# citibeth/spsparse

Hardware: AMD Instinct MI355X
Metric: nnz(C)/s for C=A*A SpGEMM (higher is better)
Workload: dtype f64

## Files before the change

### spsparse_amd/csrc/capi.hip

```cpp
#include "internal.h"

#include <cstdio>
#include <cstdlib>
#include <cstring>
#include <algorithm>
#include <exception>
#include <vector>

using namespace spsamd;

#define API_GUARD(ctx, ...)                                                         \
	if ((ctx)->busy) { (ctx)->last_error = "context busy: a streamed multiply is delivering on it"; return SPSAMD_EINVAL; } \
	try { __VA_ARGS__ }                                                             \
	catch (const spsamd::Error &e) { (ctx)->last_error = e.msg; return e.code; }    \
	catch (const std::bad_alloc &) { (ctx)->last_error = "host allocation failed"; return SPSAMD_ENOMEM; } \
	catch (const std::exception &e) { (ctx)->last_error = e.what(); return SPSAMD_EINVAL; }

extern "C" const char *spsamd_version(void) { return "spsparse_amd 0.2 (gfx950)"; }

extern "C" int spsamd_ctx_create(spsamd_ctx **out, int device, void *hip_stream)
{
	if (!out) return SPSAMD_EINVAL;
	*out = nullptr;
	int ndev = 0;
	if (hipGetDeviceCount(&ndev) != hipSuccess || ndev == 0) { (void)hipGetLastError(); return SPSAMD_ENODEVICE; }
	if (device < 0) { if (hipGetDevice(&device) != hipSuccess) return SPSAMD_ENODEVICE; }
	if (device >= ndev) return SPSAMD_ENODEVICE;
	if (hipSetDevice(device) != hipSuccess) return SPSAMD_ENODEVICE;
	spsamd_ctx *c = new (std::nothrow) spsamd_ctx();
	if (!c) return SPSAMD_ENOMEM;
	c->device = device;
	hipDeviceProp_t prop;
	if (hipGetDeviceProperties(&prop, device) == hipSuccess) c->num_cu = prop.multiProcessorCount;
	if (hip_stream) { c->stream = (hipStream_t)hip_stream; c->own_stream = false; }
	else {
		if (hipStreamCreateWithFlags(&c->stream, hipStreamNonBlocking) != hipSuccess) { delete c; return SPSAMD_EHIP; }
		c->own_stream = true;
	}
	for (auto &e : c->ev) if (hipEventCreate(&e) != hipSuccess) { spsamd_ctx_destroy(c); return SPSAMD_EHIP; }
	for (auto &e : c->ev2) if (hipEventCreate(&e) != hipSuccess) { spsamd_ctx_destroy(c); return SPSAMD_EHIP; }
	if (hipStreamCreateWithFlags(&c->side, hipStreamNonBlocking) != hipSuccess) { spsamd_ctx_destroy(c); return SPSAMD_EHIP; }
	for (auto &e : c->ev_side) if (hipEventCreateWithFlags(&e, hipEventDisableTiming) != hipSuccess) { spsamd_ctx_destroy(c); return SPSAMD_EHIP; }
	if (hipStreamCreateWithFlags(&c->side2, hipStreamNonBlocking) != hipSuccess) { spsamd_ctx_destroy(c); return SPSAMD_EHIP; }
	for (auto &e : c->ev_side2) if (hipEventCreateWithFlags(&e, hipEventDisableTiming) != hipSuccess) { spsamd_ctx_destroy(c); return SPSAMD_EHIP; }
	static const char *const knobs[] = {"window", "cell_cap", "dense_min", "no_tiles", "xcd", "emit_path", "light_path", "no_wmajor", "direct_min", "tiles_v1", "long_cap", "long_dense_min", "index_budget_mb", "trace", "light_two_pass", "spmm_path", "spmm_long_min", "add_path", "masked_path", "sampled_path", "select_path", "extract_path", "reduce_path", "emult_path", "tile_walk", "solve_path", "solve_row", "solve_fuse_rows", "factor_path", "factor_row", "factor_fuse_rows", "factor_serial_work", "factor_lds_row", "color_path", "color_row", "color_fuse_rows", "color_wave_deg"};
	static const char *const envs[] = {"SPSAMD_W", "SPSAMD_CELL_CAP", "SPSAMD_DENSE_MIN", "SPSAMD_NO_TILES", "SPSAMD_XCD", "SPSAMD_EMIT_PATH", "SPSAMD_LIGHT_PATH", "SPSAMD_NO_WMAJOR", "SPSAMD_DIRECT_MIN", "SPSAMD_TILES_V1", "SPSAMD_LONG_CAP", "SPSAMD_LONG_DENSE_MIN", "SPSAMD_INDEX_BUDGET_MB", "SPSAMD_TRACE", "SPSAMD_LIGHT_TWO_PASS", "SPSAMD_SPMM_PATH", "SPSAMD_SPMM_LONG_MIN", "SPSAMD_ADD_PATH", "SPSAMD_MASKED_PATH", "SPSAMD_SAMPLED_PATH", "SPSAMD_SELECT_PATH", "SPSAMD_EXTRACT_PATH", "SPSAMD_REDUCE_PATH", "SPSAMD_EMULT_PATH", "SPSAMD_TILE_WALK", "SPSAMD_SOLVE_PATH", "SPSAMD_SOLVE_ROW", "SPSAMD_SOLVE_FUSE_ROWS", "SPSAMD_FACTOR_PATH", "SPSAMD_FACTOR_ROW", "SPSAMD_FACTOR_FUSE_ROWS", "SPSAMD_FACTOR_SERIAL_WORK", "SPSAMD_FACTOR_LDS_ROW", "SPSAMD_COLOR_PATH", "SPSAMD_COLOR_ROW", "SPSAMD_COLOR_FUSE_ROWS", "SPSAMD_COLOR_WAVE_DEG"};
	static_assert(sizeof knobs / sizeof knobs[0] == sizeof envs / sizeof envs[0], "one environment variable per knob");
	for (size_t k = 0; k < sizeof knobs / sizeof knobs[0]; ++k)
		if (const char *e = getenv(envs[k])) (void)spsamd_ctx_set_tuning(c, knobs[k], atol(e));
#ifdef SPSAMD_ABLATIONS
	if (const char *e = getenv("SPSAMD_DBG")) c->tune.dbg = atoi(e);
#endif
	*out = c;
	return SPSAMD_OK;
}

extern "C" int spsamd_ctx_set_tuning(spsamd_ctx *c, const char *name, long value)
{
	if (!c || !name) return SPSAMD_EINVAL;
	if (c->busy) { c->last_error = "context busy: a streamed multiply is delivering on it"; return SPSAMD_EINVAL; }
	struct { const char *n; int *p; } tab[] = {
		{"window", &c->tune.window}, {"cell_cap", &c->tune.cell_cap}, {"dense_min", &c->tune.dense_min},
		{"no_tiles", &c->tune.no_tiles}, {"xcd", &c->tune.xcd}, {"emit_path", &c->tune.emit_path},
		{"light_path", &c->tune.light_path}, {"no_wmajor", &c->tune.no_wmajor}, {"direct_min", &c->tune.direct_min}, {"tiles_v1", &c->tune.tiles_v1}, {"long_cap", &c->tune.long_cap}, {"long_dense_min", &c->tune.long_dense_min}, {"index_budget_mb", &c->tune.index_budget_mb}, {"trace", &c->tune.trace}, {"light_two_pass", &c->tune.light_two_pass},
		{"spmm_path", &c->tune.spmm_path}, {"spmm_long_min", &c->tune.spmm_long_min}, {"add_path", &c->tune.add_path},
		{"masked_path", &c->tune.masked_path}, {"sampled_path", &c->tune.sampled_path}, {"select_path", &c->tune.select_path},
		{"extract_path", &c->tune.extract_path}, {"reduce_path", &c->tune.reduce_path}, {"emult_path", &c->tune.emult_path},
		{"tile_walk", &c->tune.tile_walk}, {"solve_path", &c->tune.solve_path}, {"solve_row", &c->tune.solve_row},
		{"solve_fuse_rows", &c->tune.solve_fuse_rows}, {"factor_path", &c->tune.factor_path}, {"factor_row", &c->tune.factor_row},
		{"factor_fuse_rows", &c->tune.factor_fuse_rows}, {"factor_serial_work", &c->tune.factor_serial_work},
		{"factor_lds_row", &c->tune.factor_lds_row}, {"color_path", &c->tune.color_path}, {"color_row", &c->tune.color_row},
		{"color_fuse_rows", &c->tune.color_fuse_rows}, {"color_wave_deg", &c->tune.color_wave_deg},
	};
	for (auto &t : tab) if (!std::strcmp(t.n, name)) { *t.p = (int)value; return SPSAMD_OK; }
	c->last_error = std::string("unknown tuning knob: ") + name;
	return SPSAMD_EINVAL;
}

extern "C" void spsamd_ctx_destroy(spsamd_ctx *c)
{
	if (!c) return;
	(void)hipSetDevice(c->device);
	if (c->stream) (void)hipStreamSynchronize(c->stream);
	if (c->side) (void)hipStreamSynchronize(c->side);
	if (c->side2) (void)hipStreamSynchronize(c->side2);
	c->arena.release();
	c->out[0].release(); c->out[1].release();
	c->rowstat_n.release(); c->rowstat_s.release(); c->rowstat_h.release();
	if (c->pinned) (void)hipHostFree(c->pinned);
	if (c->stream_pinned) (void)hipHostFree(c->stream_pinned);
	for (auto &e : c->ev) if (e) (void)hipEventDestroy(e);
	for (auto &e : c->ev2) if (e) (void)hipEventDestroy(e);
	for (auto &e : c->ev_side) if (e) (void)hipEventDestroy(e);
	for (auto &e : c->ev_side2) if (e) (void)hipEventDestroy(e);
	if (c->side) (void)hipStreamDestroy(c->side);
	if (c->side2) (void)hipStreamDestroy(c->side2);
	if (c->own_stream && c->stream) (void)hipStreamDestroy(c->stream);
	delete c;
}

extern "C" const char *spsamd_last_error(const spsamd_ctx *c) { return c ? c->last_error.c_str() : "null context"; }

extern "C" int spsamd_ctx_reserve(spsamd_ctx *c, size_t workspace_bytes, size_t output_tuples)
{
	if (!c) return SPSAMD_EINVAL;
	API_GUARD(c,
		SPS_HIP(hipSetDevice(c->device));
		if (workspace_bytes) c->arena.reserve(workspace_bytes);
		if (output_tuples) {
			OutSet &o = c->out[c->cur_out];
			o.i.ensure(output_tuples * sizeof(int32_t));
			o.j.ensure(output_tuples * sizeof(int32_t));
			o.v.ensure(output_tuples * sizeof(double));
		}
		return SPSAMD_OK;
	)
}

bool spsamd::same_operand(const spsamd_coo *a, const spsamd_coo *b)
{
	return a->idx0 == b->idx0 && a->idx1 == b->idx1 && a->val == b->val && a->nnz == b->nnz &&
		a->shape0 == b->shape0 && a->shape1 == b->shape1 && a->sort0 == b->sort0 && a->mem == b->mem;
}

int spsamd::multiply_body(spsamd_ctx *c, double C,
	const spsamd_vec *scalei, const spsamd_coo *A, char transpose_A,
	const spsamd_vec *scalej, const spsamd_coo *B, char transpose_B,
	const spsamd_vec *scalek, int duplicate_policy, int zero_nan,
	int sink_kind, int sink_flags, spsamd_result *res, const char *what, bool arena_ready, const OperandParts *parts, bool b_rank1)
{
	check_sink_args(duplicate_policy, sink_kind);
	std::memset(res, 0, sizeof(*res));
	const bool permute = (sink_flags & SPSAMD_SINK_PERMUTE) && sink_kind == SPSAMD_SINK_COO;
	const ProductFrame f(A, transpose_A, B, transpose_B, permute);
	const int a0 = f.a0, bk = f.bk, bj = f.bj;
	res->shape0 = f.shape0; res->shape1 = f.shape1;
	f.check_inner(what);
	if (product_is_empty(C, scalei, A, scalej, B, scalek)) return SPSAMD_OK;

	SPS_HIP(hipSetDevice(c->device));
	if (!arena_ready) c->arena.reset();
	hipStream_t st = c->stream;
	SPS_HIP(hipEventRecord(c->ev[EV_BEGIN], st));
	{ const spsamd_coo *ops[2] = {A, B}; pick_output_set(c, ops, 2); }
	MultiplyArgs a;
	a.C = C; a.sink_kind = sink_kind; a.sink_flags = sink_flags;
	if (parts) { a.pa = parts->pa; a.pb = parts->pb; a.b_ready = parts->b_ready; a.static_walk = true; }
	Prepared *hp = nullptr;
	consolidate_operand(c, A, a0, a0, duplicate_policy, zero_nan, &a.A, &hp);
	if (hp) a.pa = hp;
	if (a0 == bk && same_operand(A, B) && (!zero_nan || hp)) { a.B = a.A; if (a.pa) a.pb = a.pa; }
	else { consolidate_operand(c, B, bk, b_rank1 ? bk : bj, duplicate_policy, zero_nan, &a.B, &hp); if (hp) a.pb = hp; }
	if (sink_kind == SPSAMD_SINK_COO) c->own[c->cur_out].sort0 = -1;
	upload_scale(c, scalei, f.nrow, "scalei", &a.si);
	upload_scale(c, scalej, f.inner, "scalej", &a.sj);
// ... 462 lines not shown
```

### spsparse_amd/csrc/internal.h

```cpp
#pragma once

#include <hip/hip_runtime.h>
#include <stdint.h>
#include <stddef.h>
#include <string>
#include <vector>

#include "../../include/spsparse_amd.h"

namespace spsamd {


struct Error {
	int code;
	std::string msg;
};

#define SPS_HIP(call)                                                              \
	do {                                                                           \
		hipError_t e_ = (call);                                                    \
		if (e_ != hipSuccess)                                                      \
			throw ::spsamd::Error{SPSAMD_EHIP, std::string(#call) + ": " + hipGetErrorString(e_)}; \
	} while (0)

#define SPS_LAUNCH_CHECK() SPS_HIP(hipGetLastError())


struct Arena {
	struct Slab { char *p; size_t cap; size_t used; };
	std::vector<Slab> slabs;
	size_t high_water = 0;
	size_t call_used = 0;

	void *alloc(size_t bytes);
	struct Mark { size_t nslabs, used, call_used; };
	Mark mark() const { return Mark{slabs.size(), slabs.empty() ? 0 : slabs.back().used, call_used}; }
	void rewind(const Mark &m);
	void reset();
	void release();
	void reserve(size_t bytes);
	template <class T> T *get(size_t n) { return (T *)alloc(n * sizeof(T)); }
};

struct DevBuf {
	void *p = nullptr;
	size_t cap = 0;
	void ensure(size_t bytes);
	void release();
	bool holds(const void *q) const { return p && q && (const char *)q >= (const char *)p && (const char *)q < (const char *)p + cap; }
};

struct OutSet {
	DevBuf i, j, v;
	bool holds(const void *q) const { return i.holds(q) || j.holds(q) || v.holds(q); }
	void release() { i.release(); j.release(); v.release(); }
};

struct Tuning {
	int window = 0;
	int cell_cap = 0;
	int dense_min = 0;
	int no_tiles = 0;
	int xcd = 2;
	int emit_path = 0;
	int light_path = 0;
	int light_two_pass = 0;
	int no_wmajor = 0;
	int tiles_v1 = 0;
	int long_cap = 0;
	int long_dense_min = 0;
	int direct_min = 0;
	int trace = 0;
	int index_budget_mb = 0;
	int spmm_path = 0;
	int spmm_long_min = 0;
	int add_path = 0;
	int masked_path = 0;
	int sampled_path = 0;
	int select_path = 0;
	int extract_path = 0;
	int reduce_path = 0;
	int tile_walk = 0;
	int emult_path = 0;
	int solve_path = 0;
	int solve_row = 0;
	int solve_fuse_rows = 0;
	int factor_path = 0;
	int factor_row = 0;
	int factor_fuse_rows = 0;
	int factor_serial_work = 0;
	int factor_lds_row = 0;
	int color_path = 0;
	int color_row = 0;
	int color_fuse_rows = 0;
	int color_wave_deg = 0;
#ifdef SPSAMD_ABLATIONS
	int dbg = 0;
#endif
};
}

struct spsamd_ctx {
	int device = 0;
	spsamd::Tuning tune;
	hipStream_t stream = nullptr;
	bool own_stream = false;
	spsamd::Arena arena;
	spsamd::OutSet out[2];
	int cur_out = 0;
	struct OwnResult { const int32_t *d0 = nullptr, *d1 = nullptr; const double *v = nullptr; uint64_t nnz = 0, shape0 = 0, shape1 = 0; int sort0 = -1; } own[2];
	spsamd::DevBuf rowstat_n, rowstat_s, rowstat_h;
	void *pinned = nullptr;
	size_t pinned_cap = 0;
	std::string last_error;
	hipEvent_t ev[10] = {};
	hipEvent_t ev2[3] = {};
	hipStream_t side = nullptr;
	hipEvent_t ev_side[2] = {};
	hipStream_t side2 = nullptr;
	hipEvent_t ev_side2[2] = {};
	bool wm_pending = false, sort_pending = false;
	void join_side(bool wm, bool sort);
	int num_cu = 256;
	void *host_staging(size_t bytes);
	bool busy = false;
	void *stream_pinned = nullptr;
	size_t stream_pinned_cap = 0;
};

namespace spsamd {

struct SideScope {
	SideScope(spsamd_ctx *c, int which, bool record_fork);
	~SideScope();
	SideScope(const SideScope &) = delete;
	SideScope &operator=(const SideScope &) = delete;
private:
	spsamd_ctx *c;
	hipStream_t main, side;
	hipEvent_t join;
};

enum Ev {
	EV_NONE = -1,
	EV_BEGIN = 0,
	EV_CONSOLIDATED = 1,
	EV_SYMBOLIC = 2,
	EV_N0 = 3,
	EV_N1 = 4,
	EV_N2 = 5,
	EV_N3 = 6,
	EV_END = 7,
	EV_N4 = 8,
// ... 328 lines not shown
```

### spsparse_amd/csrc/k_dense.hip

```cpp
#include "spgemm_host.h"
#include "bank_layout.h"

namespace spsamd {


#ifndef DENSE_SCAN_BATCH
#define DENSE_SCAN_BATCH 8
#endif
#ifndef DENSE_SCAN_XCHG
#define DENSE_SCAN_XCHG 1
#endif
template <int W, int NT, int MODE, bool PAT, bool PLAIN>
__global__ __launch_bounds__(NT, 4) void k_dense(const Cell *cells, uint32_t ncell, const uint32_t *xb, RowMeta m,
	const uint32_t *widx, uint64_t kstride, uint64_t wstride, uint32_t narrow, EmitParams ep, SinkParams sk, uint32_t *claim_ctr)
{
	constexpr int NW = NT / 64;
	constexpr int NGRP = W / 64;
	constexpr int GPW = NGRP / NW;
	constexpr uint32_t WSHIFT = W == 8192 ? 13 : 14;
	constexpr int R = DENSE_R;
	constexpr int NWORD = W / 64;
	constexpr int WPL = NWORD / 64;
	constexpr int SB = DENSE_SCAN_BATCH < GPW ? DENSE_SCAN_BATCH : GPW;
	static_assert(GPW % SB == 0, "whole batches");
	static_assert(!PLAIN || (!PAT && MODE != MODE_COUNT), "PLAIN: STORE and DIGEST without EXACT_PATTERN");
	__shared__ double acc[MODE == MODE_COUNT ? 1 : W + 64];
	__shared__ __attribute__((aligned(16))) uint8_t ctouch[MODE == MODE_COUNT ? W : 16];
	__shared__ uint32_t s_cpref[NT + 1];
	__shared__ uint2 s_cse[NT];
	__shared__ double s_caval[NT];
	__shared__ unsigned long long s_bmask[NWORD];
	__shared__ uint32_t s_scrL[2][NW], s_scrN[2][NW];
	__shared__ uint32_t s_wcnt[NW + 1];
	__shared__ PatCell s_pat;
	__shared__ unsigned long long s_u64[2 * NW];
	__shared__ double s_f64[NW];
	__shared__ uint32_t s_claim[4];

	const unsigned tid = threadIdx.x, lane = lane_id();
	const unsigned wv = (unsigned)__builtin_amdgcn_readfirstlane((int)wave_id());
	const double CLEAN = (PAT && MODE != MODE_COUNT) ? -0.0 : 0.0;
	if (MODE == MODE_COUNT) { for (int q = tid; q < W / 16; q += NT) reinterpret_cast<uint4 *>(ctouch)[q] = make_uint4(0, 0, 0, 0); }
	else for (int q = tid; q < W + 64; q += NT) acc[q] = CLEAN;
	for (int q = tid; q < NWORD; q += NT) s_bmask[q] = 0ull;
	const bool plain = PLAIN || (PAT && emit_plain(ep));
	const unsigned long long laneK = (unsigned long long)lane * 0x9E3779B97F4A7C15ull;
	unsigned long long d_cnt = 0, d_hash = 0; double d_sum = 0;
	PatAcc pat; pat_init(pat);
	if (tid == 0) pat_reset(&s_pat);
	uint32_t flip = 0;
	STAMP_BEGIN();

	constexpr uint32_t NONE = 0xFFFFFFFFu;
	const bool claimed = claim_ctr != nullptr && xb != nullptr && !ABL(ep, 16);
	const CellWalk walk = cell_walk(claimed ? nullptr : xb, ncell);
	const uint32_t stride = walk.stride, cend = walk.end;
	const uint32_t clast = ncell ? ncell - 1 : 0;
	uint32_t part = blockIdx.x & 7u, tried = 0;
	auto claim_resolve = [&](uint32_t got) -> uint32_t {
		while (true) {
			if (got < xb[part + 1]) return got;
			if (++tried >= 8u) return NONE;
			part = (part + 1u) & 7u;
			got = atomicAdd(&claim_ctr[part * 32u], 1u);
		}
	};
	uint32_t i0, i1, i2;
	if (claimed) {
		if (tid == 0) {
			for (int q = 0; q < 3; ++q) s_claim[q] = tried >= 8u ? NONE : claim_resolve(atomicAdd(&claim_ctr[part * 32u], 1u));
			s_claim[3] = NONE;
		}
		__syncthreads();
		i0 = s_claim[0]; i1 = s_claim[1]; i2 = NONE;
	} else {
		i0 = walk.first < cend ? walk.first : NONE;
		i1 = i0 != NONE && i0 + stride < cend ? i0 + stride : NONE;
		i2 = i1 != NONE && i1 + stride < cend ? i1 + stride : NONE;
	}
	i0 = (uint32_t)__builtin_amdgcn_readfirstlane((int)i0); i1 = (uint32_t)__builtin_amdgcn_readfirstlane((int)i1); i2 = (uint32_t)__builtin_amdgcn_readfirstlane((int)i2);
	const uint32_t zlane = cell_pend_zero();
	Cell rec1 = cells[min(i0, clast)];
	CellPend pend2 = cell_pend_load(cells, min(i1, clast), zlane);
	uint32_t nlo, nlen; double na;
	auto seg_bounds = [&](int32_t k, uint32_t w, uint32_t &lo, uint32_t &hi) {
		const uint32_t *bw = widx + (uint64_t)(uint32_t)k * kstride + (uint64_t)w * wstride;
		lo = bw[0]; hi = bw[1];
	};
	{
		const uint32_t e = rec1.beg + tid;
		const bool act = i0 != NONE && e < rec1.end;
		const uint32_t ec = e < rec1.end ? e : rec1.beg;
		uint32_t lo, hi;
		seg_bounds(m.acol[ec], rec1.wa, lo, hi);
		na = m.aval[ec];
		nlo = lo; nlen = act ? hi - lo : 0u;
	}
	int32_t nkA; double naA;
	{
		const uint32_t e1 = rec1.beg + NT + tid;
		const uint32_t e1c = e1 < rec1.end ? e1 : rec1.beg;
		nkA = m.acol[e1c]; naA = m.aval[e1c];
	}
	__syncthreads();
	uint32_t iter = 0;
	for (; i0 != NONE; ++iter, i0 = i1, i1 = i2, i2 = (claimed || i2 == NONE || i2 + stride >= cend) ? (claimed ? i2 : NONE) : i2 + stride) {
		const Cell cell = rec1;
		const uint32_t w = cell.wa;
		const uint32_t beg = cell.beg, end = cell.end;
		const int32_t rowid = cell.rowid;
		double a_scale = 1.0;
		if constexpr (!PLAIN) a_scale = row_scale(ep, rowid);
		const uint32_t wbase = w << WSHIFT;
		uint32_t lo = nlo, len = nlen; double a = na;
		rec1 = cell_from_pend(pend2);
		if (!claimed) pend2 = cell_pend_load(cells, min(i2, clast), zlane);
		const uint32_t ne = rec1.beg + tid;
		const bool nact = i1 != NONE && ne < rec1.end;
		const uint32_t nec = ne < rec1.end ? ne : rec1.beg;
		const int32_t nk = m.acol[nec];
		na = m.aval[nec];
		int32_t kA = nkA; double aA = naA;
		{
			const uint32_t e1 = rec1.beg + NT + tid;
			const uint32_t e1c = e1 < rec1.end ? e1 : rec1.beg;
			nkA = m.acol[e1c]; naA = m.aval[e1c];
		}

		STAMP_COUNT(8);
		uint32_t pnseg = 0;
		for (uint32_t chunk = beg; chunk < end; chunk += NT) {
			STAMP_COUNT(9);
			uint32_t lo2, hi2; double a2;
			{
				seg_bounds(kA, w, lo2, hi2);
				a2 = aA;
				if (chunk + NT + tid >= end) hi2 = lo2;
				const uint32_t e2 = chunk + 2 * NT + tid;
				const uint32_t e2c = e2 < end ? e2 : beg;
				kA = m.acol[e2c]; aA = m.aval[e2c];
			}
			const uint32_t items = (len + R - 1) / R;
			const uint32_t inc = wave_inclusive_scan_u32(items);
			const uint64_t nzm = __ballot(len != 0);
			const uint32_t wrank = (uint32_t)__popcll(nzm & lanemask_lt());
			if (lane == 63) s_scrL[flip][wv] = inc;
			if (lane == 0) s_scrN[flip][wv] = (uint32_t)__popcll(nzm);
			STAMP(0);
			lds_barrier();
			STAMP(1);
			if (claimed && chunk == beg) {
				i2 = (uint32_t)__builtin_amdgcn_readfirstlane((int)s_claim[2 + (iter & 1u)]);
				pend2 = cell_pend_load(cells, min(i2, clast), zlane);
			}
			uint32_t baseL = 0, baseN = 0, total = 0, nzc = 0;
#pragma unroll
			for (int q = 0; q < NW; ++q) {
				const uint32_t l = s_scrL[flip][q], n = s_scrN[flip][q];
				if (q < (int)wv) { baseL += l; baseN += n; }
				total += l; nzc += n;
			}
			flip ^= 1u;
			total = (uint32_t)__builtin_amdgcn_readfirstlane((int)total);
			nzc = (uint32_t)__builtin_amdgcn_readfirstlane((int)nzc);
			const uint32_t myfirst = baseL + inc - items;
			if (len) {
				const uint32_t rank = baseN + wrank;
				s_cpref[rank] = myfirst;
				s_cse[rank] = make_uint2(lo, lo + len);
				s_caval[rank] = a;
				if (myfirst < (uint32_t)W) atomicOr(reinterpret_cast<uint32_t *>(s_bmask) + (myfirst >> 5), 1u << (myfirst & 31u));
			}
			if (ABL(ep, 8)) total = 0;
			if (total == 0) { lo = lo2; len = hi2 - lo2; a = a2; continue; }
			if (ep.ordered && MODE != MODE_COUNT) {
				lds_barrier();
				for (uint32_t q = 0; q < nzc; ++q) {
					const uint2 se = s_cse[q];
					const double aq = s_caval[q];
					for (uint32_t t = se.x + tid; t < se.y; t += NT) {
						const BTup bt = m.btup[t];
						const uint32_t slot = dense_phys((uint32_t)bt.col - wbase);
						acc[slot] = acc[slot] + aq * btup_val(bt);
					}
					lds_barrier();
				}
				for (int q = tid; q < NWORD; q += NT) s_bmask[q] = 0ull;
				lo = lo2; len = hi2 - lo2; a = a2;
				continue;
			}
			uint32_t Q0 = 0;
			for (uint32_t pb = 0; pb < total; pb += W) {
				const uint32_t pe = min(total, pb + (uint32_t)W);
				if (pb) {
					lds_barrier();
					for (int q = tid; q < NWORD; q += NT) s_bmask[q] = 0ull;
					lds_barrier();
					if (len && myfirst >= pb && myfirst < pe) atomicOr(&s_bmask[(myfirst - pb) >> 6], 1ull << ((myfirst - pb) & 63u));
				}
				STAMP(2);
				lds_barrier();
				STAMP(3);
				unsigned long long mw[WPL]; uint32_t pre[WPL];
				uint32_t run = Q0;
#pragma unroll
				for (int x = 0; x < WPL; ++x) {
					mw[x] = s_bmask[x * 64 + lane];
					const uint32_t cnt = (uint32_t)__popcll(mw[x]);
					const uint32_t incl = wave_inclusive_scan_u32(cnt);
					pre[x] = run + incl - cnt;
					run += (uint32_t)__builtin_amdgcn_readlane((int)incl, 63);
				}
				const uint32_t nsteps = (pe - pb + NT - 1) / NT;
				auto lookup = [&](uint32_t step, uint32_t &obp, uint32_t &onv, double &oav) {
					const uint32_t b = step * NW + wv;
					const uint32_t t = pb + (b << 6) + lane;
					const bool ok = t < pe;
					uint32_t mlo = 0, mhi = 0, pr = 0;
#pragma unroll
					for (int x = 0; x < WPL; ++x) {
						if ((b >> 6) == (uint32_t)x) {
							mlo = (uint32_t)__builtin_amdgcn_readlane((int)(uint32_t)mw[x], (int)(b & 63u));
							mhi = (uint32_t)__builtin_amdgcn_readlane((int)(uint32_t)(mw[x] >> 32), (int)(b & 63u));
							pr = (uint32_t)__builtin_amdgcn_readlane((int)pre[x], (int)(b & 63u));
						}
					}
					if (ABL(ep, 128)) { obp = (t * R) & 0xFFFFFu; onv = ok ? R : 0u; oav = 1.0; return; }
					const uint32_t s1lo = (mlo >> 1) | (mhi << 31), s1hi = mhi >> 1;
					const uint32_t qs = pr + (mlo & 1u) - 1u;
					uint32_t q = qs + __builtin_amdgcn_mbcnt_hi(s1hi, __builtin_amdgcn_mbcnt_lo(s1lo, 0u));
					q = min(q, nzc - 1u);
					const uint2 se = s_cse[q];
					obp = se.x + (t - s_cpref[q]) * R;
					onv = ok ? min((uint32_t)R, se.y - obp) : 0u;
					oav = s_caval[q];
				};
				const char *bbase = reinterpret_cast<const char *>(m.btup);
				auto fetch = [&](uint32_t bp_) -> BPiece {
					if (ABL(ep, 64)) bp_ &= 0xFFFFu;
					if (narrow) return *reinterpret_cast<const BPiece *>(bbase + (uint32_t)((bp_ << 3) + (bp_ << 2)));
					return *reinterpret_cast<const BPiece *>(bbase + (uint64_t)bp_ * 12u);
				};
				auto accumulate = [&](const BPiece &piece, uint32_t nv_, double av_) {
#pragma unroll
					for (int u = 0; u < R; ++u) {
						const uint32_t col = ABL(ep, 64) ? (piece.w[3 * u] & (W - 1)) : piece.w[3 * u] - wbase;
						const uint32_t slot = (uint32_t)u < nv_ ? (MODE == MODE_COUNT ? col : dense_phys(col)) : (uint32_t)W + lane;
						if (ABL(ep, 32)) { if (piece.w[3 * u + 2] == 0x7FF12345u) acc[MODE == MODE_COUNT ? 0 : slot] = av_; }
						else if (MODE == MODE_COUNT) { if ((uint32_t)u < nv_) ctouch[slot] = (uint8_t)1; }
						else {
							const double pv = av_ * __hiloint2double((int)piece.w[3 * u + 2], (int)piece.w[3 * u + 1]);
							atomicAdd(&acc[slot], pv);
							if (PAT && (uint32_t)u < nv_) pat_note(pat, pv);
						}
					}
				};
				STAMP(4);
#if DENSE_DEPTH == 2
				uint32_t bp0, nv0, bp1 = 0, nv1 = 0; double av0, av1 = 0.0;
				lookup(0, bp0, nv0, av0);
				BPiece p0 = fetch(bp0), p1 = p0;
				if (nsteps > 1) lookup(1, bp1, nv1, av1);
				for (uint32_t step = 0; step < nsteps; ++step) {
					STAMP_COUNT(10);
					if (step + 1 < nsteps) p1 = fetch(bp1);
					uint32_t bp2 = 0, nv2 = 0; double av2 = 0.0;
					if (step + 2 < nsteps) lookup(step + 2, bp2, nv2, av2);
					accumulate(p0, nv0, av0);
					p0 = p1; nv0 = nv1; av0 = av1;
					bp1 = bp2; nv1 = nv2; av1 = av2;
				}
#else
				uint32_t bp, nv; double av;
				lookup(0, bp, nv, av);
				for (uint32_t step = 0; step < nsteps; ++step) {
					STAMP_COUNT(10);
					const BPiece piece = fetch(bp);
					uint32_t nbp = bp, nnv = 0; double nav = 0.0;
					if (step + 1 < nsteps) lookup(step + 1, nbp, nnv, nav);
					accumulate(piece, nv, av);
					bp = nbp; nv = nnv; av = nav;
				}
#endif
				Q0 = run;
				STAMP(5);
			}
			if (PAT) { pat_publish(pat, &s_pat); pnseg += nzc; }
			lds_barrier();
			STAMP(6);
			for (int q = tid; q < NWORD; q += NT) s_bmask[q] = 0ull;
			lo = lo2; len = hi2 - lo2; a = a2;
		}
		{
			uint32_t l2, h2;
			seg_bounds(nk, rec1.wa, l2, h2);
			nlo = l2; nlen = nact ? h2 - l2 : 0u;
		}
		if (ABL(ep, 16)) continue;
		STAMP(0);
		uint32_t claim_pending = NONE;
		if (claimed && tid == 0 && tried < 8u) claim_pending = atomicAdd(&claim_ctr[part * 32u], 1u);
		const double pthr = PAT ? pat_threshold(&s_pat, pnseg) : -1.0;
		const uint32_t pbeg = beg, pend = end;
		double v[MODE == MODE_STORE ? GPW : 1];
		uint64_t nzmask[MODE == MODE_STORE ? GPW : 1];
		uint32_t wcount = 0;
		constexpr unsigned long long MIXK = 0x9E3779B97F4A7C15ull;
		unsigned long long X0 = ((((unsigned long long)(uint32_t)rowid) << 32) | (unsigned long long)(wbase + wv * GPW * 64u)) * MIXK;
		X0 = ((unsigned long long)(uint32_t)__builtin_amdgcn_readfirstlane((int)(uint32_t)(X0 >> 32)) << 32) |
			(unsigned long long)(uint32_t)__builtin_amdgcn_readfirstlane((int)(uint32_t)X0);
		double r_sum = 0;
		unsigned long long r_hash = 0;
		if constexpr (MODE == MODE_COUNT) {
			static_assert(W / 16 == NT, "sixteen flag bytes per thread");
			uint32_t cnt = 0;
			{
				uint4 *cw = reinterpret_cast<uint4 *>(ctouch);
				const uint4 x = cw[tid];
				const uint32_t xs[4] = {x.x, x.y, x.z, x.w};
				if (x.x | x.y | x.z | x.w) {
					cw[tid] = make_uint4(0, 0, 0, 0);
#pragma unroll
					for (int q = 0; q < 4; ++q) {
						if (!ep.sk_pos) cnt += (uint32_t)__popc(xs[q]);
						else {
#pragma unroll
							for (int b = 0; b < 4; ++b)
								if (((xs[q] >> (8 * b)) & 1u) && col_allowed(ep, (int32_t)(wbase + tid * 16u + (uint32_t)(4 * q + b)))) ++cnt;
						}
					}
				}
			}
			wcount = (uint32_t)wave_reduce_sum((unsigned long long)cnt);
		} else {
		auto slot_of = [&](int gi) -> uint32_t {
			const int grp = wv * GPW + gi;
			return grp * 64 + (lane ^ (uint32_t)__builtin_amdgcn_readfirstlane((int)dense_swz((uint32_t)grp)));
		};
		double xs[SB];
#pragma unroll
		for (int gi = 0; gi < GPW; ++gi) {
			if (gi % SB == 0) {
#if DENSE_SCAN_XCHG
				unsigned long long *acc64 = reinterpret_cast<unsigned long long *>(acc);
#pragma unroll
				for (int q = 0; q < SB; ++q) xs[q] = __longlong_as_double((long long)atomicExch(&acc64[slot_of(gi + q)], (unsigned long long)__double_as_longlong(CLEAN)));
#else
#pragma unroll
				for (int q = 0; q < SB; ++q) xs[q] = acc[slot_of(gi + q)];
#pragma unroll
				for (int q = 0; q < SB; ++q) acc[slot_of(gi + q)] = CLEAN;
#endif
				__builtin_amdgcn_sched_barrier(0);
			}
			const int grp = wv * GPW + gi;
			const int32_t col = (int32_t)(wbase + grp * 64 + lane);
			double x = xs[gi % SB];
			if (PAT) {
				const bool touched = __double_as_longlong(x) != (long long)0x8000000000000000ull;
				x = pat_fix_wave(touched && !(fabs(x) > pthr), x, col, m, pbeg, pend);
			}
			const bool ok = emit_test<PLAIN>(plain, ep, a_scale, col, x);
			const uint64_t mk = __ballot(ok);
			wcount += (uint32_t)__popcll(mk);
			if (MODE == MODE_STORE) { v[gi] = x; nzmask[gi] = mk; }
			if (MODE == MODE_DIGEST) {
				unsigned long long h = X0 + laneK;
				h ^= h >> 29;
				r_hash += ok ? h : 0ull;
				if (plain && !PAT) r_sum += x;
				else r_sum += ok ? x : 0.0;
				X0 += 64ull * MIXK;
			}
		}
		}
		if (MODE == MODE_DIGEST) {
			if (lane == 0) d_cnt += wcount;
			d_sum += r_sum;
			d_hash += r_hash;
			if (sk.row_nnz) {
				double rs = wave_reduce_sum(r_sum);
				r_hash = wave_reduce_sum(r_hash);
				if (lane == 0 && wcount) { atomicAdd((unsigned long long *)&sk.row_nnz[rowid], (unsigned long long)wcount); atomicAdd(&sk.row_sum[rowid], rs); atomicAdd(&sk.row_hash[rowid], r_hash); }
			}
		} else {
			if (lane == 0) s_wcnt[wv] = wcount;
			__syncthreads();
			uint32_t wbefore = 0, wtotal = 0;
#pragma unroll
			for (int q = 0; q < NW; ++q) { uint32_t t = s_wcnt[q]; if (q < (int)wv) wbefore += t; wtotal += t; }
			if (MODE == MODE_COUNT) {
				if (tid == 0) sk.segcount[cell.seg] = wtotal;
			} else {
				int64_t o = sk.segoff[cell.seg] + wbefore;
#pragma unroll
				for (int gi = 0; gi < GPW; ++gi) {
					uint64_t mk = nzmask[gi];
					if ((mk >> lane) & 1ull) {
						int64_t oo = o + __popcll(mk & lanemask_lt());
						sk.out_i[oo] = rowid;
						sk.out_j[oo] = (int32_t)(wbase + (wv * GPW + gi) * 64 + lane);
						sk.out_v[oo] = v[gi];
					}
					o += __popcll(mk);
				}
				if (tid == 0) sk.segactual[cell.seg] = wtotal;
			}
			__syncthreads();
		}
		STAMP(7);
		if (PAT) { lds_barrier(); if (tid == 0) pat_reset(&s_pat); }
		if (claimed && tid == 0) s_claim[2 + ((iter + 1u) & 1u)] = tried < 8u ? claim_resolve(claim_pending) : NONE;
	}
	STAMP_FLUSH();
	if (MODE == MODE_DIGEST) digest_flush<NT>(sk.digest, d_cnt, d_hash, d_sum, s_u64, s_f64);
}

__global__ void k_claim_init(const uint32_t *xb, uint32_t *ctr)
{
	if (threadIdx.x < 8) ctr[threadIdx.x * 32u] = xb[threadIdx.x];
}

template <int MODE>
void launch_heavy_dense(spsamd_ctx *c, const Heavy &hv, const RowMeta &m0, const EmitParams &ep, const SinkParams &sk)
{
	if (!hv.ncell[CLS_DENSE]) return;
	uint32_t *claim = nullptr;
	if (c->tune.xcd == 2 && hv.xb[CLS_DENSE]) {
		claim = c->arena.get<uint32_t>(8 * 32);
		k_claim_init<<<dim3(1), dim3(64), 0, c->stream>>>(hv.xb[CLS_DENSE], claim);
		SPS_LAUNCH_CHECK();
	}
	RowMeta m = m0;
	const uint32_t *widx = hv.bwin;
	uint64_t kstride = hv.nwin1, wstride = 1;
	if (hv.wptr) { widx = hv.wptr; kstride = 1; wstride = hv.nrowb; m.btup = hv.btw; }
	const uint32_t narrow = hv.narrow();
	unsigned grid = std::min<unsigned>(hv.ncell[CLS_DENSE], (unsigned)c->num_cu * (hv.W != 8192 ? 1u : (MODE == MODE_COUNT ? 3u : 2u)));
	if (grid >= 64) grid &= ~7u;
	const SinkParams &sks = stamps_sink(c, sk, grid);
	auto go = [&](auto w, auto nt, auto pat, auto pln) {
		k_dense<decltype(w)::value, decltype(nt)::value, MODE, decltype(pat)::value, decltype(pln)::value><<<dim3(grid), dim3(decltype(nt)::value), 0, c->stream>>>(hv.cells[CLS_DENSE], hv.ncell[CLS_DENSE], hv.xb[CLS_DENSE], m, widx, kstride, wstride, narrow, ep, sks, claim);
	};
	auto go_pat = [&](auto w, auto nt) {
		if (ep.pattern) return go(w, nt, std::true_type{}, std::false_type{});
		if constexpr (MODE != MODE_COUNT) { if (emit_plain(ep)) return go(w, nt, std::false_type{}, std::true_type{}); }
		go(w, nt, std::false_type{}, std::false_type{});
	};
	if (hv.W == 8192) go_pat(std::integral_constant<int, 8192>{}, std::integral_constant<int, 512>{});
	else go_pat(std::integral_constant<int, 16384>{}, std::integral_constant<int, 1024>{});
	SPS_LAUNCH_CHECK();
	static const char *const nm[11] = {"pre-B1", "B1wait", "compact", "B2wait", "tables", "steps", "B3wait", "scanout", "cells", "chunks", "steps#"};
	stamps_report(c, sks, grid, "k_dense", nm, 11, 8);
}

template void launch_heavy_dense<MODE_COUNT>(spsamd_ctx *, const Heavy &, const RowMeta &, const EmitParams &, const SinkParams &);
template void launch_heavy_dense<MODE_STORE>(spsamd_ctx *, const Heavy &, const RowMeta &, const EmitParams &, const SinkParams &);
template void launch_heavy_dense<MODE_DIGEST>(spsamd_ctx *, const Heavy &, const RowMeta &, const EmitParams &, const SinkParams &);

}
```

Before: 163.1 billion.

## Batch multiple A-chunks into one dense expansion group with double-buffered bitmask

New measurement: 164.4 billion (median of 6 runs). No clear change (+0.8%).

```diff
diff --git a/spsparse_amd/csrc/capi.hip b/spsparse_amd/csrc/capi.hip
--- a/spsparse_amd/csrc/capi.hip
+++ b/spsparse_amd/csrc/capi.hip
@@ -43,8 +43,8 @@
 	for (auto &e : c->ev_side) if (hipEventCreateWithFlags(&e, hipEventDisableTiming) != hipSuccess) { spsamd_ctx_destroy(c); return SPSAMD_EHIP; }
 	if (hipStreamCreateWithFlags(&c->side2, hipStreamNonBlocking) != hipSuccess) { spsamd_ctx_destroy(c); return SPSAMD_EHIP; }
 	for (auto &e : c->ev_side2) if (hipEventCreateWithFlags(&e, hipEventDisableTiming) != hipSuccess) { spsamd_ctx_destroy(c); return SPSAMD_EHIP; }
-	static const char *const knobs[] = {"window", "cell_cap", "dense_min", "no_tiles", "xcd", "emit_path", "light_path", "no_wmajor", "direct_min", "tiles_v1", "long_cap", "long_dense_min", "index_budget_mb", "trace", "light_two_pass", "spmm_path", "spmm_long_min", "add_path", "masked_path", "sampled_path", "select_path", "extract_path", "reduce_path", "emult_path", "tile_walk", "solve_path", "solve_row", "solve_fuse_rows", "factor_path", "factor_row", "factor_fuse_rows", "factor_serial_work", "factor_lds_row", "color_path", "color_row", "color_fuse_rows", "color_wave_deg"};
-	static const char *const envs[] = {"SPSAMD_W", "SPSAMD_CELL_CAP", "SPSAMD_DENSE_MIN", "SPSAMD_NO_TILES", "SPSAMD_XCD", "SPSAMD_EMIT_PATH", "SPSAMD_LIGHT_PATH", "SPSAMD_NO_WMAJOR", "SPSAMD_DIRECT_MIN", "SPSAMD_TILES_V1", "SPSAMD_LONG_CAP", "SPSAMD_LONG_DENSE_MIN", "SPSAMD_INDEX_BUDGET_MB", "SPSAMD_TRACE", "SPSAMD_LIGHT_TWO_PASS", "SPSAMD_SPMM_PATH", "SPSAMD_SPMM_LONG_MIN", "SPSAMD_ADD_PATH", "SPSAMD_MASKED_PATH", "SPSAMD_SAMPLED_PATH", "SPSAMD_SELECT_PATH", "SPSAMD_EXTRACT_PATH", "SPSAMD_REDUCE_PATH", "SPSAMD_EMULT_PATH", "SPSAMD_TILE_WALK", "SPSAMD_SOLVE_PATH", "SPSAMD_SOLVE_ROW", "SPSAMD_SOLVE_FUSE_ROWS", "SPSAMD_FACTOR_PATH", "SPSAMD_FACTOR_ROW", "SPSAMD_FACTOR_FUSE_ROWS", "SPSAMD_FACTOR_SERIAL_WORK", "SPSAMD_FACTOR_LDS_ROW", "SPSAMD_COLOR_PATH", "SPSAMD_COLOR_ROW", "SPSAMD_COLOR_FUSE_ROWS", "SPSAMD_COLOR_WAVE_DEG"};
+	static const char *const knobs[] = {"window", "cell_cap", "dense_min", "no_tiles", "xcd", "emit_path", "light_path", "no_wmajor", "direct_min", "tiles_v1", "long_cap", "long_dense_min", "index_budget_mb", "trace", "light_two_pass", "spmm_path", "spmm_long_min", "add_path", "masked_path", "sampled_path", "select_path", "extract_path", "reduce_path", "emult_path", "tile_walk", "solve_path", "solve_row", "solve_fuse_rows", "factor_path", "factor_row", "factor_fuse_rows", "factor_serial_work", "factor_lds_row", "color_path", "color_row", "color_fuse_rows", "color_wave_deg", "dense_groups"};
+	static const char *const envs[] = {"SPSAMD_W", "SPSAMD_CELL_CAP", "SPSAMD_DENSE_MIN", "SPSAMD_NO_TILES", "SPSAMD_XCD", "SPSAMD_EMIT_PATH", "SPSAMD_LIGHT_PATH", "SPSAMD_NO_WMAJOR", "SPSAMD_DIRECT_MIN", "SPSAMD_TILES_V1", "SPSAMD_LONG_CAP", "SPSAMD_LONG_DENSE_MIN", "SPSAMD_INDEX_BUDGET_MB", "SPSAMD_TRACE", "SPSAMD_LIGHT_TWO_PASS", "SPSAMD_SPMM_PATH", "SPSAMD_SPMM_LONG_MIN", "SPSAMD_ADD_PATH", "SPSAMD_MASKED_PATH", "SPSAMD_SAMPLED_PATH", "SPSAMD_SELECT_PATH", "SPSAMD_EXTRACT_PATH", "SPSAMD_REDUCE_PATH", "SPSAMD_EMULT_PATH", "SPSAMD_TILE_WALK", "SPSAMD_SOLVE_PATH", "SPSAMD_SOLVE_ROW", "SPSAMD_SOLVE_FUSE_ROWS", "SPSAMD_FACTOR_PATH", "SPSAMD_FACTOR_ROW", "SPSAMD_FACTOR_FUSE_ROWS", "SPSAMD_FACTOR_SERIAL_WORK", "SPSAMD_FACTOR_LDS_ROW", "SPSAMD_COLOR_PATH", "SPSAMD_COLOR_ROW", "SPSAMD_COLOR_FUSE_ROWS", "SPSAMD_COLOR_WAVE_DEG", "SPSAMD_DENSE_GROUPS"};
 	static_assert(sizeof knobs / sizeof knobs[0] == sizeof envs / sizeof envs[0], "one environment variable per knob");
 	for (size_t k = 0; k < sizeof knobs / sizeof knobs[0]; ++k)
 		if (const char *e = getenv(envs[k])) (void)spsamd_ctx_set_tuning(c, knobs[k], atol(e));
@@ -71,6 +71,7 @@
 		{"factor_fuse_rows", &c->tune.factor_fuse_rows}, {"factor_serial_work", &c->tune.factor_serial_work},
 		{"factor_lds_row", &c->tune.factor_lds_row}, {"color_path", &c->tune.color_path}, {"color_row", &c->tune.color_row},
 		{"color_fuse_rows", &c->tune.color_fuse_rows}, {"color_wave_deg", &c->tune.color_wave_deg},
+		{"dense_groups", &c->tune.dense_groups},
 	};
 	for (auto &t : tab) if (!std::strcmp(t.n, name)) { *t.p = (int)value; return SPSAMD_OK; }
 	c->last_error = std::string("unknown tuning knob: ") + name;
diff --git a/spsparse_amd/csrc/internal.h b/spsparse_amd/csrc/internal.h
--- a/spsparse_amd/csrc/internal.h
+++ b/spsparse_amd/csrc/internal.h
@@ -69,6 +69,7 @@
 	int tiles_v1 = 0;
 	int long_cap = 0;
 	int long_dense_min = 0;
+	int dense_groups = 0;
 	int direct_min = 0;
 	int trace = 0;
 	int index_budget_mb = 0;
diff --git a/spsparse_amd/csrc/k_dense.hip b/spsparse_amd/csrc/k_dense.hip
--- a/spsparse_amd/csrc/k_dense.hip
+++ b/spsparse_amd/csrc/k_dense.hip
@@ -12,7 +12,7 @@
 #endif
 template <int W, int NT, int MODE, bool PAT, bool PLAIN>
 __global__ __launch_bounds__(NT, 4) void k_dense(const Cell *cells, uint32_t ncell, const uint32_t *xb, RowMeta m,
-	const uint32_t *widx, uint64_t kstride, uint64_t wstride, uint32_t narrow, EmitParams ep, SinkParams sk, uint32_t *claim_ctr)
+	const uint32_t *widx, uint64_t kstride, uint64_t wstride, uint32_t narrow, uint32_t one_chunk, EmitParams ep, SinkParams sk, uint32_t *claim_ctr)
 {
 	constexpr int NW = NT / 64;
 	constexpr int NGRP = W / 64;
@@ -29,7 +29,7 @@
 	__shared__ uint32_t s_cpref[NT + 1];
 	__shared__ uint2 s_cse[NT];
 	__shared__ double s_caval[NT];
-	__shared__ unsigned long long s_bmask[NWORD];
+	__shared__ unsigned long long s_bmask[2][NWORD];
 	__shared__ uint32_t s_scrL[2][NW], s_scrN[2][NW];
 	__shared__ uint32_t s_wcnt[NW + 1];
 	__shared__ PatCell s_pat;
@@ -42,13 +42,14 @@
 	const double CLEAN = (PAT && MODE != MODE_COUNT) ? -0.0 : 0.0;
 	if (MODE == MODE_COUNT) { for (int q = tid; q < W / 16; q += NT) reinterpret_cast<uint4 *>(ctouch)[q] = make_uint4(0, 0, 0, 0); }
 	else for (int q = tid; q < W + 64; q += NT) acc[q] = CLEAN;
-	for (int q = tid; q < NWORD; q += NT) s_bmask[q] = 0ull;
+	for (int q = tid; q < NWORD; q += NT) { s_bmask[0][q] = 0ull; s_bmask[1][q] = 0ull; }
 	const bool plain = PLAIN || (PAT && emit_plain(ep));
 	const unsigned long long laneK = (unsigned long long)lane * 0x9E3779B97F4A7C15ull;
 	unsigned long long d_cnt = 0, d_hash = 0; double d_sum = 0;
 	PatAcc pat; pat_init(pat);
 	if (tid == 0) pat_reset(&s_pat);
 	uint32_t flip = 0;
+	uint32_t buf = 0;
 	STAMP_BEGIN();
 
 	constexpr uint32_t NONE = 0xFFFFFFFFu;
@@ -96,11 +97,11 @@
 		na = m.aval[ec];
 		nlo = lo; nlen = act ? hi - lo : 0u;
 	}
-	int32_t nkA; double naA;
+	int32_t nkA;
 	{
 		const uint32_t e1 = rec1.beg + NT + tid;
 		const uint32_t e1c = e1 < rec1.end ? e1 : rec1.beg;
-		nkA = m.acol[e1c]; naA = m.aval[e1c];
+		nkA = m.acol[e1c];
 	}
 	__syncthreads();
 	uint32_t iter = 0;
@@ -120,26 +121,31 @@
 		const uint32_t nec = ne < rec1.end ? ne : rec1.beg;
 		const int32_t nk = m.acol[nec];
 		na = m.aval[nec];
-		int32_t kA = nkA; double aA = naA;
+		int32_t kA = nkA;
 		{
 			const uint32_t e1 = rec1.beg + NT + tid;
 			const uint32_t e1c = e1 < rec1.end ? e1 : rec1.beg;
-			nkA = m.acol[e1c]; naA = m.aval[e1c];
+			nkA = m.acol[e1c];
 		}
 
 		STAMP_COUNT(8);
 		uint32_t pnseg = 0;
+		uint32_t gseg = 0, gitems = 0;
+		uint32_t lo2, hi2; double a2;
+		auto ahead = [&](uint32_t chunk) {
+			seg_bounds(kA, w, lo2, hi2);
+			const uint32_t e1 = chunk + NT + tid, e2 = e1 + NT;
+			a2 = m.aval[e1 < end ? e1 : beg];
+			kA = m.acol[e2 < end ? e2 : beg];
+		};
+		auto advance = [&](uint32_t chunk) {
+			lo = lo2; len = chunk + NT + tid < end ? hi2 - lo2 : 0u; a = a2;
+			asm volatile("" : "+v"(lo), "+v"(len), "+v"(a) :: "memory");
+			if (chunk + NT < end) ahead(chunk + NT);
+		};
+		ahead(beg);
 		for (uint32_t chunk = beg; chunk < end; chunk += NT) {
 			STAMP_COUNT(9);
-			uint32_t lo2, hi2; double a2;
-			{
-				seg_bounds(kA, w, lo2, hi2);
-				a2 = aA;
-				if (chunk + NT + tid >= end) hi2 = lo2;
-				const uint32_t e2 = chunk + 2 * NT + tid;
-				const uint32_t e2c = e2 < end ? e2 : beg;
-				kA = m.acol[e2c]; aA = m.aval[e2c];
-			}
 			const uint32_t items = (len + R - 1) / R;
 			const uint32_t inc = wave_inclusive_scan_u32(items);
 			const uint64_t nzm = __ballot(len != 0);
@@ -164,16 +170,19 @@
 			total = (uint32_t)__builtin_amdgcn_readfirstlane((int)total);
 			nzc = (uint32_t)__builtin_amdgcn_readfirstlane((int)nzc);
 			const uint32_t myfirst = baseL + inc - items;
-			if (len) {
-				const uint32_t rank = baseN + wrank;
-				s_cpref[rank] = myfirst;
-				s_cse[rank] = make_uint2(lo, lo + len);
-				s_caval[rank] = a;
-				if (myfirst < (uint32_t)W) atomicOr(reinterpret_cast<uint32_t *>(s_bmask) + (myfirst >> 5), 1u << (myfirst & 31u));
-			}
+			auto put = [&](uint32_t sbase, uint32_t ibase) {
+				if (len) {
+					const uint32_t rank = sbase + baseN + wrank, first = ibase + myfirst;
+					s_cpref[rank] = first;
+					s_cse[rank] = make_uint2(lo, lo + len);
+					s_caval[rank] = a;
+					if (first < (uint32_t)W) atomicOr(reinterpret_cast<uint32_t *>(s_bmask[buf]) + (first >> 5), 1u << (first & 31u));
+				}
+			};
 			if (ABL(ep, 8)) total = 0;
-			if (total == 0) { lo = lo2; len = hi2 - lo2; a = a2; continue; }
 			if (ep.ordered && MODE != MODE_COUNT) {
+				put(0u, 0u);
+				if (total == 0) { advance(chunk); continue; }
 				lds_barrier();
 				for (uint32_t q = 0; q < nzc; ++q) {
 					const uint2 se = s_cse[q];
@@ -185,111 +194,124 @@
 					}
 					lds_barrier();
 				}
-				for (int q = tid; q < NWORD; q += NT) s_bmask[q] = 0ull;
-				lo = lo2; len = hi2 - lo2; a = a2;
+				for (int q = tid; q < NWORD; q += NT) s_bmask[buf][q] = 0ull;
+				advance(chunk);
 				continue;
 			}
-			uint32_t Q0 = 0;
-			for (uint32_t pb = 0; pb < total; pb += W) {
-				const uint32_t pe = min(total, pb + (uint32_t)W);
-				if (pb) {
-					lds_barrier();
-					for (int q = tid; q < NWORD; q += NT) s_bmask[q] = 0ull;
-					lds_barrier();
-					if (len && myfirst >= pb && myfirst < pe) atomicOr(&s_bmask[(myfirst - pb) >> 6], 1ull << ((myfirst - pb) & 63u));
+			const bool lastc = chunk + NT >= end;
+			auto run = [&](const bool fresh) __attribute__((always_inline)) {
+				STAMP_COUNT(11);
+				unsigned long long *const bm = s_bmask[buf];
+				uint32_t Q0 = 0;
+				for (uint32_t pb = 0; pb < gitems; pb += W) {
+					const uint32_t pe = min(gitems, pb + (uint32_t)W);
+					if (pb) {
+						lds_barrier();
+						for (int q = tid; q < NWORD; q += NT) bm[q] = 0ull;
+						lds_barrier();
+						if (len && myfirst >= pb && myfirst < pe) atomicOr(&bm[(myfirst - pb) >> 6], 1ull << ((myfirst - pb) & 63u));
+					}
+					STAMP(2);
+					if (fresh || pb) lds_barrier();
+					STAMP(3);
+					unsigned long long mw[WPL]; uint32_t pre[WPL];
+					uint32_t run = Q0;
+#pragma unroll
+					for (int x = 0; x < WPL; ++x) {
+						mw[x] = bm[x * 64 + lane];
+						const uint32_t cnt = (uint32_t)__popcll(mw[x]);
+						const uint32_t incl = wave_inclusive_scan_u32(cnt);
+						pre[x] = run + incl - cnt;
+						run += (uint32_t)__builtin_amdgcn_readlane((int)incl, 63);
+					}
+					const uint32_t nsteps = (pe - pb + NT - 1) / NT;
+					auto lookup = [&](uint32_t step, uint32_t &obp, uint32_t &onv, double &oav) {
+						const uint32_t b = step * NW + wv;
+						const uint32_t t = pb + (b << 6) + lane;
+						const bool ok = t < pe;
+						uint32_t mlo = 0, mhi = 0, pr = 0;
+#pragma unroll
+						for (int x = 0; x < WPL; ++x) {
+							if ((b >> 6) == (uint32_t)x) {
+								mlo = (uint32_t)__builtin_amdgcn_readlane((int)(uint32_t)mw[x], (int)(b & 63u));
+								mhi = (uint32_t)__builtin_amdgcn_readlane((int)(uint32_t)(mw[x] >> 32), (int)(b & 63u));
+								pr = (uint32_t)__builtin_amdgcn_readlane((int)pre[x], (int)(b & 63u));
+							}
+						}
+						if (ABL(ep, 128)) { obp = (t * R) & 0xFFFFFu; onv = ok ? R : 0u; oav = 1.0; return; }
+						const uint32_t s1lo = (mlo >> 1) | (mhi << 31), s1hi = mhi >> 1;
+						const uint32_t qs = pr + (mlo & 1u) - 1u;
+						uint32_t q = qs + __builtin_amdgcn_mbcnt_hi(s1hi, __builtin_amdgcn_mbcnt_lo(s1lo, 0u));
+						q = min(q, gseg - 1u);
+						const uint2 se = s_cse[q];
+						obp = se.x + (t - s_cpref[q]) * R;
+						onv = ok ? min((uint32_t)R, se.y - obp) : 0u;
+						oav = s_caval[q];
+					};
+					const char *bbase = reinterpret_cast<const char *>(m.btup);
+					auto fetch = [&](uint32_t bp_) -> BPiece {
+						if (ABL(ep, 64)) bp_ &= 0xFFFFu;
+						if (narrow) return *reinterpret_cast<const BPiece *>(bbase + (uint32_t)((bp_ << 3) + (bp_ << 2)));
+						return *reinterpret_cast<const BPiece *>(bbase + (uint64_t)bp_ * 12u);
+					};
+					auto accumulate = [&](const BPiece &piece, uint32_t nv_, double av_) {
+#pragma unroll
+						for (int u = 0; u < R; ++u) {
+							const uint32_t col = ABL(ep, 64) ? (piece.w[3 * u] & (W - 1)) : piece.w[3 * u] - wbase;
+							const uint32_t slot = (uint32_t)u < nv_ ? (MODE == MODE_COUNT ? col : dense_phys(col)) : (uint32_t)W + lane;
+							if (ABL(ep, 32)) { if (piece.w[3 * u + 2] == 0x7FF12345u) acc[MODE == MODE_COUNT ? 0 : slot] = av_; }
+							else if (MODE == MODE_COUNT) { if ((uint32_t)u < nv_) ctouch[slot] = (uint8_t)1; }
+							else {
+								const double pv = av_ * __hiloint2double((int)piece.w[3 * u + 2], (int)piece.w[3 * u + 1]);
+								atomicAdd(&acc[slot], pv);
+								if (PAT && (uint32_t)u < nv_) pat_note(pat, pv);
+							}
+						}
+					};
+					STAMP(4);
+#if DENSE_DEPTH == 2
+					uint32_t bp0, nv0, bp1 = 0, nv1 = 0; double av0, av1 = 0.0;
+					lookup(0, bp0, nv0, av0);
+					BPiece p0 = fetch(bp0), p1 = p0;
+					if (nsteps > 1) lookup(1, bp1, nv1, av1);
+					for (uint32_t step = 0; step < nsteps; ++step) {
+						STAMP_COUNT(10);
+						if (step + 1 < nsteps) p1 = fetch(bp1);
+						uint32_t bp2 = 0, nv2 = 0; double av2 = 0.0;
+						if (step + 2 < nsteps) lookup(step + 2, bp2, nv2, av2);
+						accumulate(p0, nv0, av0);
+						p0 = p1; nv0 = nv1; av0 = av1;
+						bp1 = bp2; nv1 = nv2; av1 = av2;
+					}
+#else
+					uint32_t bp, nv; double av;
+					lookup(0, bp, nv, av);
+					for (uint32_t step = 0; step < nsteps; ++step) {
+						STAMP_COUNT(10);
+						const BPiece piece = fetch(bp);
+						uint32_t nbp = bp, nnv = 0; double nav = 0.0;
+						if (step + 1 < nsteps) lookup(step + 1, nbp, nnv, nav);
+						accumulate(piece, nv, av);
+						bp = nbp; nv = nnv; av = nav;
+					}
+#endif
+					Q0 = run;
+					STAMP(5);
 				}
+				if (PAT) { pat_publish(pat, &s_pat); pnseg += gseg; }
+				lds_barrier();
+				STAMP(6);
+				for (int q = tid; q < NWORD; q += NT) bm[q] = 0ull;
+				buf ^= 1u; gseg = 0u; gitems = 0u;
+			};
+			if (total != 0u) {
+				if (gseg != 0u && (total > (uint32_t)W || gseg + nzc > (uint32_t)NT || gitems + total > (uint32_t)W)) run(false);
+				put(gseg, gitems);
+				gseg += nzc; gitems += total;
 				STAMP(2);
-				lds_barrier();
-				STAMP(3);
-				unsigned long long mw[WPL]; uint32_t pre[WPL];
-				uint32_t run = Q0;
-#pragma unroll
-				for (int x = 0; x < WPL; ++x) {
-					mw[x] = s_bmask[x * 64 + lane];
-					const uint32_t cnt = (uint32_t)__popcll(mw[x]);
-					const uint32_t incl = wave_inclusive_scan_u32(cnt);
-					pre[x] = run + incl - cnt;
-					run += (uint32_t)__builtin_amdgcn_readlane((int)incl, 63);
-				}
-				const uint32_t nsteps = (pe - pb + NT - 1) / NT;
-				auto lookup = [&](uint32_t step, uint32_t &obp, uint32_t &onv, double &oav) {
-					const uint32_t b = step * NW + wv;
-					const uint32_t t = pb + (b << 6) + lane;
-					const bool ok = t < pe;
-					uint32_t mlo = 0, mhi = 0, pr = 0;
-#pragma unroll
-					for (int x = 0; x < WPL; ++x) {
-						if ((b >> 6) == (uint32_t)x) {
-							mlo = (uint32_t)__builtin_amdgcn_readlane((int)(uint32_t)mw[x], (int)(b & 63u));
-							mhi = (uint32_t)__builtin_amdgcn_readlane((int)(uint32_t)(mw[x] >> 32), (int)(b & 63u));
-							pr = (uint32_t)__builtin_amdgcn_readlane((int)pre[x], (int)(b & 63u));
-						}
-					}
-					if (ABL(ep, 128)) { obp = (t * R) & 0xFFFFFu; onv = ok ? R : 0u; oav = 1.0; return; }
-					const uint32_t s1lo = (mlo >> 1) | (mhi << 31), s1hi = mhi >> 1;
-					const uint32_t qs = pr + (mlo & 1u) - 1u;
-					uint32_t q = qs + __builtin_amdgcn_mbcnt_hi(s1hi, __builtin_amdgcn_mbcnt_lo(s1lo, 0u));
-					q = min(q, nzc - 1u);
-					const uint2 se = s_cse[q];
-					obp = se.x + (t - s_cpref[q]) * R;
-					onv = ok ? min((uint32_t)R, se.y - obp) : 0u;
-					oav = s_caval[q];
-				};
-				const char *bbase = reinterpret_cast<const char *>(m.btup);
-				auto fetch = [&](uint32_t bp_) -> BPiece {
-					if (ABL(ep, 64)) bp_ &= 0xFFFFu;
-					if (narrow) return *reinterpret_cast<const BPiece *>(bbase + (uint32_t)((bp_ << 3) + (bp_ << 2)));
-					return *reinterpret_cast<const BPiece *>(bbase + (uint64_t)bp_ * 12u);
-				};
-				auto accumulate = [&](const BPiece &piece, uint32_t nv_, double av_) {
-#pragma unroll
-					for (int u = 0; u < R; ++u) {
-						const uint32_t col = ABL(ep, 64) ? (piece.w[3 * u] & (W - 1)) : piece.w[3 * u] - wbase;
-						const uint32_t slot = (uint32_t)u < nv_ ? (MODE == MODE_COUNT ? col : dense_phys(col)) : (uint32_t)W + lane;
-						if (ABL(ep, 32)) { if (piece.w[3 * u + 2] == 0x7FF12345u) acc[MODE == MODE_COUNT ? 0 : slot] = av_; }
-						else if (MODE == MODE_COUNT) { if ((uint32_t)u < nv_) ctouch[slot] = (uint8_t)1; }
-						else {
-							const double pv = av_ * __hiloint2double((int)piece.w[3 * u + 2], (int)piece.w[3 * u + 1]);
-							atomicAdd(&acc[slot], pv);
-							if (PAT && (uint32_t)u < nv_) pat_note(pat, pv);
-						}
-					}
-				};
-				STAMP(4);
-#if DENSE_DEPTH == 2
-				uint32_t bp0, nv0, bp1 = 0, nv1 = 0; double av0, av1 = 0.0;
-				lookup(0, bp0, nv0, av0);
-				BPiece p0 = fetch(bp0), p1 = p0;
-				if (nsteps > 1) lookup(1, bp1, nv1, av1);
-				for (uint32_t step = 0; step < nsteps; ++step) {
-					STAMP_COUNT(10);
-					if (step + 1 < nsteps) p1 = fetch(bp1);
-					uint32_t bp2 = 0, nv2 = 0; double av2 = 0.0;
-					if (step + 2 < nsteps) lookup(step + 2, bp2, nv2, av2);
-					accumulate(p0, nv0, av0);
-					p0 = p1; nv0 = nv1; av0 = av1;
-					bp1 = bp2; nv1 = nv2; av1 = av2;
-				}
-#else
-				uint32_t bp, nv; double av;
-				lookup(0, bp, nv, av);
-				for (uint32_t step = 0; step < nsteps; ++step) {
-					STAMP_COUNT(10);
-					const BPiece piece = fetch(bp);
-					uint32_t nbp = bp, nnv = 0; double nav = 0.0;
-					if (step + 1 < nsteps) lookup(step + 1, nbp, nnv, nav);
-					accumulate(piece, nv, av);
-					bp = nbp; nv = nnv; av = nav;
-				}
-#endif
-				Q0 = run;
-				STAMP(5);
-			}
-			if (PAT) { pat_publish(pat, &s_pat); pnseg += nzc; }
-			lds_barrier();
-			STAMP(6);
-			for (int q = tid; q < NWORD; q += NT) s_bmask[q] = 0ull;
-			lo = lo2; len = hi2 - lo2; a = a2;
+				if (lastc || one_chunk || gitems > (uint32_t)W) run(true);
+			} else if (lastc && gseg != 0u) run(false);
+			advance(chunk);
 		}
 		{
 			uint32_t l2, h2;
@@ -436,11 +458,12 @@
 	uint64_t kstride = hv.nwin1, wstride = 1;
 	if (hv.wptr) { widx = hv.wptr; kstride = 1; wstride = hv.nrowb; m.btup = hv.btw; }
 	const uint32_t narrow = hv.narrow();
+	const uint32_t one_chunk = c->tune.dense_groups == 1 ? 1u : 0u;
 	unsigned grid = std::min<unsigned>(hv.ncell[CLS_DENSE], (unsigned)c->num_cu * (hv.W != 8192 ? 1u : (MODE == MODE_COUNT ? 3u : 2u)));
 	if (grid >= 64) grid &= ~7u;
 	const SinkParams &sks = stamps_sink(c, sk, grid);
 	auto go = [&](auto w, auto nt, auto pat, auto pln) {
-		k_dense<decltype(w)::value, decltype(nt)::value, MODE, decltype(pat)::value, decltype(pln)::value><<<dim3(grid), dim3(decltype(nt)::value), 0, c->stream>>>(hv.cells[CLS_DENSE], hv.ncell[CLS_DENSE], hv.xb[CLS_DENSE], m, widx, kstride, wstride, narrow, ep, sks, claim);
+		k_dense<decltype(w)::value, decltype(nt)::value, MODE, decltype(pat)::value, decltype(pln)::value><<<dim3(grid), dim3(decltype(nt)::value), 0, c->stream>>>(hv.cells[CLS_DENSE], hv.ncell[CLS_DENSE], hv.xb[CLS_DENSE], m, widx, kstride, wstride, narrow, one_chunk, ep, sks, claim);
 	};
 	auto go_pat = [&](auto w, auto nt) {
 		if (ep.pattern) return go(w, nt, std::true_type{}, std::false_type{});
@@ -450,8 +473,8 @@
 	if (hv.W == 8192) go_pat(std::integral_constant<int, 8192>{}, std::integral_constant<int, 512>{});
 	else go_pat(std::integral_constant<int, 16384>{}, std::integral_constant<int, 1024>{});
 	SPS_LAUNCH_CHECK();
-	static const char *const nm[11] = {"pre-B1", "B1wait", "compact", "B2wait", "tables", "steps", "B3wait", "scanout", "cells", "chunks", "steps#"};
-	stamps_report(c, sks, grid, "k_dense", nm, 11, 8);
+	static const char *const nm[12] = {"pre-B1", "B1wait", "compact", "B2wait", "tables", "steps", "B3wait", "scanout", "cells", "chunks", "steps#", "groups"};
+	stamps_report(c, sks, grid, "k_dense", nm, 12, 8);
 }
 
 template void launch_heavy_dense<MODE_COUNT>(spsamd_ctx *, const Heavy &, const RowMeta &, const EmitParams &, const SinkParams &);
```
